# hritikbharucha/Custom_Porechop_ABI

Measured on AMD Instinct MI355X. Metric: reads/sec trimmed (100k ONT reads x 50 adapter pairs), higher is better.
Workload: dtype int32

## Files before the change

custom_porechop_abi_amd/csrc/pcabi_dp.h:

```cpp
#pragma once

#ifndef PCABI_ROW_FENCE
#define PCABI_ROW_FENCE 1
#endif
#ifndef PCABI_TAB_PD
#define PCABI_TAB_PD 0
#endif
#ifndef PCABI_TAB_PD_LONG
#define PCABI_TAB_PD_LONG 1
#endif

#include <stdint.h>
#include <algorithm>

#ifdef __HIPCC__
#define PCABI_HD __host__ __device__ __forceinline__
#else
#define PCABI_HD inline
#endif

namespace pcabi {

constexpr int NEG = -(1 << 28);

// ... 450 lines not shown
    st.best.b.trail = 0;
    st.best.b.precd = 0;
    st.best.c = -L;
    st.best.n = 0;
    st.bc = st.best;
    st.bc.b.score = SCORE_FLOOR;
    st.cslt = LT_NONE;
    st.cvt = 0;
    st.cvp = 0;
#pragma unroll 1
    for (int k = k0; k < nst; ++k) {
        adp.load(k);
        const bool first = k == k0, fin = k == nst - 1;
        const int off = first ? pad - k0 * R : 0;
        const int ib = k * R - pad;
        st.init_stripe(ib, off);
        ReadFn rd = rd0;
        BndCell up, nx, bot;
        auto row0 = [](int j, BndCell &u) { u.s = 0; u.v = NEG; u.sc = j; u.vc = 0; u.sn = 0; u.vn = 0; };
        if (first) row0(1, up);
        else bnd.load(1, up);
        int r = rd(1);
#pragma unroll 1
        for (int j = 1; j < n; ++j) {
            const int rn = rd(j + 1);
            if (first) row0(j + 1, nx);
            else bnd.load(j + 1, nx);
            st.template column<false>(r, j, up, adp, off, ib, L, fin, j >= own_lo && j < hi, sc, bot);
            if (!fin) bnd.store(j, bot);
            up = nx;
            r = rn;
        }
        if (fin_read) st.template column<true>(r, n, up, adp, off, ib, L, fin, n >= own_lo && n < hi, sc, bot);
        else st.template column<false>(r, n, up, adp, off, ib, L, fin, n >= own_lo && n < hi, sc, bot);
        if (!fin) bnd.store(n, bot);
    }
    return finish_path(st.best.b, st.best.c, (int)(st.best.n & 0xFFFFu), (int)(st.best.n >> 16), L,
                       fin_read ? n : n + 1);
}

}

namespace pcabi {

constexpr uint32_t INC_PAD = 1u << ATTR_CSH;

PCABI_HD int32_t vreg(int32_t x) {
#if defined(__HIP_DEVICE_COMPILE__)
    asm volatile("" : "+v"(x));
#endif
    return x;
}

PCABI_HD int max3i(int a, int b, int c) {
    const int ab = a > b ? a : b;
    return ab > c ? ab : c;
}
constexpr int PAD_CODE = 5;

template <int RPL, bool AFFINE>
struct LaneDP {
    int S[RPL + 1], H[RPL + 1];
    uint32_t SA[RPL + 1], HA[RPL + 1];
    int bscore, bi, bj, blt, btrail, bprec;
    uint32_t battr;
    int slt_last, ht_last, hp_last;
    int mis[4];
    uint32_t ids[4];

    template <typename AdpFn, bool LAST>
    PCABI_HD void column(const int r, const int j, const AdpFn &adp, const int L, const int off,
                         const Scoring &sc) {
        int sup = 0, vup = NEG;
        uint32_t saup = attr_start(j), vaup = 0;
        int slt_up = LT_NONE, vt_up = 0, vp_up = 0;
        int lv = 0, lh = 0, ls = 0, lslt = LT_D;
        bool lhext = false;
        uint32_t lva = 0, lha = 0, lsa = 0;
        bool match = (r == adp(1));
        int diag = 0 + (match ? sc.ma : mis[1]);
        uint32_t da = attr_start(j - 1) + ids[1] + (uint32_t)match;
#pragma unroll
        for (int s = 1; s <= RPL; ++s) {
            int diag_nx = 0;
            uint32_t da_nx = 0;
            if (s < RPL) {
                const bool mt = (r == adp(s + 1));
                const int mi_n = (s + 1 <= 3) ? mis[s + 1] : sc.mi;
                const uint32_t id_n = (s + 1 <= 3) ? ids[s + 1] : INC_D;
                diag_nx = S[s] + (mt ? sc.ma : mi_n);
                da_nx = SA[s] + id_n + (uint32_t)mt;
            }
            int hn, vn, sn;
            uint32_t han, van;
            bool hext, vext, fromv;
            if (AFFINE) {
                const int hx = H[s] + sc.ge, ho = S[s] + sc.go;
                hext = !(hx < ho);
                hn = hext ? hx : ho;
                han = hext ? HA[s] : SA[s];
                const int vx = vup + sc.ge, vo = sup + sc.go;
                vext = !(vx < vo);
                vn = vext ? vx : vo;
                van = vext ? vaup : saup;
            } else {
                hext = vext = false;
// ... 567 lines not shown
    }
    n_fin = n;
    if (CHUNK && own_hi >= 0) {
        st.template column<decltype(tabfn(r)), false, true>(tabfn(r), n, L, off, n >= own_lo && n < hi);
        st.materialize(L);
        n_fin = n + 1;
    } else {
        st.materialize(L);
        st.template column<decltype(tabfn(r)), true>(tabfn(r), n, L, off);
    }
    Best b;
    b.score = st.bscore; b.bi = st.bi; b.bj = st.bj; b.attr = Y::to_std(st.battr, st.bj);
    b.ltype = st.blt; b.trail = st.btrail; b.precd = st.bprec;
    return b;
}

template <int RPL, bool AFFINE, bool CHUNK = false, typename Y = pk::Lay<RPL>, typename ReadFn, typename TabFn>
PCABI_HD Result align_lane_packed(ReadFn &rd, int n, const TabFn &tabfn, int L, const Scoring sc, int own_lo = 1,
                                  int own_hi = -1) {
    int n_fin;
    const Best b = packed_best<RPL, AFFINE, CHUNK, Y>(rd, n, tabfn, L, sc, own_lo, own_hi, n_fin);
    return finish(b, L, n_fin);
}

namespace pk {
template <int RPL, typename AdpFn>
PCABI_HD int32_t sub_key_shift(int s, int c, const AdpFn &adp, int off, const Scoring &sc) {
    using Y = LayS<RPL>;
    if (s <= off) return Y::TD_K + Y::sc(-sc.go - sc.ge);
    return (c == adp(s)) ? (Y::sc(sc.ma - sc.go - sc.ge) + Y::TD_K + Y::INC_M)
                         : (Y::sc(sc.mi - sc.go - sc.ge) + Y::TD_K + Y::INC_D);
}
template <typename TabRow>
struct ShiftRow {
    TabRow t;
    int32_t d;
    PCABI_HD int32_t operator()(int s) const { return addw(t(s), d); }
    PCABI_HD void quad(int q, int32_t *dst) const {
        t.quad(q, dst);
        for (int k = 0; k < 4; ++k) dst[k] = addw(dst[k], d);
    }
};
}

template <int RPL, int PD = PCABI_TAB_PD>
struct LaneShift {
    using Y = pk::LayS<RPL>;
    LanePacked<RPL, true, pk::LayT<RPL>, PD> st;
    int32_t kgo;
    int32_t ftop;
    int32_t k_e;
    int32_t k_eR;
    int32_t k_rb;
    int jj, P;

    PCABI_HD void init(int L, const Scoring &sc, int P_, int B) {
        using pk::addw;
        const int off = RPL - L;
        P = P_;
        jj = 0;
        k_e = Y::sc(-sc.ge);
        k_eR = Y::sc(-sc.ge * RPL);
        k_rb = Y::sc(sc.ge * P);
        ftop = Y::sc(-B);
        kgo = Y::sc(sc.go - sc.ge) + ((P - 1) << Y::TB_SH);
        int32_t fs = addw(ftop, kgo);
#pragma unroll
        for (int s = 1; s <= RPL; ++s) {
            fs = addw(fs, k_e);
            st.G[s] = addw(Y::start(off - s), fs);
            st.HK[s] = addw(fs, Y::sc(-1) + Y::TAG1);
        }
        st.bkey = Y::start(-L);
        st.bj = 0;
    }

    PCABI_HD void advance() {
        using pk::addw;
        ++jj;
        kgo -= Y::TAG1;
        ftop = addw(ftop, k_e);
        if (jj == P) {
            const int32_t rb = addw(k_rb, P << Y::TB_SH);
#pragma unroll
            for (int s = 1; s <= RPL; ++s) {
                st.G[s] = addw(st.G[s], rb);
                st.HK[s] = addw(st.HK[s], rb);
            }
            jj = 0;
            kgo += P << Y::TB_SH;
            ftop = addw(ftop, k_rb);
        }
    }

    template <typename TabRow>
    PCABI_HD void column(const TabRow &tab, const int j, const int off) {
        using pk::addw;
        const int32_t kg = vreg(kgo);
        const int32_t top = addw(ftop, kgo);
        int32_t gup = addw(Y::start(j + off), top);
        int32_t vup = Y::SENT;
        int32_t diag = addw(addw(Y::start(j - 1 + off), top), Y::TAG1 - k_e);
        constexpr int NQ = RPL / 4;
        int32_t t[RPL + 2];
        if (PD > 0) {
#pragma unroll
            for (int q = 0; q <= PD && q < NQ; ++q) tab.quad(q, t + 4 * q + 1);
        }
        diag += (PD > 0 ? t[1] : tab(1));
        int32_t lv = 0, ls = 0;
#pragma unroll
        for (int s = 1; s <= RPL; ++s) {
            if (PD > 0 && (s & 3) == 1) {
                const int q = (s - 1) / 4 + PD + 1;
                if (q < NQ) tab.quad(q, t + 4 * q + 1);
            }
            int32_t diag_nx = 0;
            if (s < RPL) diag_nx = st.G[s] + (PD > 0 ? t[s + 1] : tab(s + 1));
            const int32_t hn = std::max(st.HK[s], st.G[s]);
            const int32_t vo = gup + Y::kv(s);
            const int32_t vn = std::max(vup, vo);
            const int32_t sn = max3i(diag, vn, hn);
            if (s == RPL) { lv = vn; ls = sn; }
            st.G[s] = (sn & ~Y::TAGM) + kg;
            st.HK[s] = hn;
            gup = st.G[s];
            vup = vn;
            diag = diag_nx;
#if defined(__HIP_DEVICE_COMPILE__)
            if (PCABI_ROW_FENCE > 0 && (s % (PCABI_ROW_FENCE > 0 ? PCABI_ROW_FENCE : 1)) == 0) __builtin_amdgcn_sched_barrier(0);
#endif
        }
        const int32_t corr = addw(std::max(lv, ls & ~Y::TAGM), pk::negw(addw(ftop, k_eR)));
        const bool upd = corr > (st.bkey | ((1 << Y::SC_SH) - 1));
        st.bkey = upd ? corr : st.bkey;
        st.bj = upd ? j : st.bj;
    }

    PCABI_HD void to_layt(const Scoring &sc) {
        using pk::addw;
        using pk::negw;
        const int32_t tagA = kgo - Y::sc(sc.go - sc.ge);
        int32_t cg = addw(negw(addw(ftop, kgo)), Y::sc(sc.go));
        int32_t ch = negw(addw(ftop, tagA + Y::TAG1));
#pragma unroll
        for (int s = 1; s <= RPL; ++s) {
            cg = addw(cg, negw(k_e));
            ch = addw(ch, negw(k_e));
            st.G[s] = addw(st.G[s], cg);
            st.HK[s] = addw(st.HK[s], ch);
        }
    }
};

template <int RPL, int PD = PCABI_TAB_PD, typename ReadFn, typename TabFn>
PCABI_HD Result align_lane_shift(ReadFn &rd, int n, const TabFn &tabfn, int L, const Scoring sc, int P, int B) {
    using Y = pk::LayS<RPL>;
    LaneShift<RPL, PD> ls;
    const int off = RPL - L;
    ls.init(L, sc, P, B);
    int r = rd(1);
#pragma unroll 1
    for (int j = 1; j < n; ++j) {
        const int rn = rd(j + 1);
        ls.advance();
        ls.template column<decltype(tabfn(r))>(tabfn(r), j, off);
        r = rn;
    }
    ls.to_layt(sc);
    auto &st = ls.st;
    const int32_t neg = Y::sc(pk::neg_score(sc));
    st.k_ge = vreg(Y::sc(sc.ge));
    st.k_go = vreg(Y::sc(sc.go));
    st.k_gev = st.k_geh = 0;
    st.k_gex = vreg(Y::sc(sc.ge) + Y::TB1);
    st.k_vo = Y::TB2;
    st.neg2 = neg | Y::TB2;
    st.materialize(L);
    const pk::ShiftRow<decltype(tabfn(r))> row{tabfn(r), Y::sc(sc.ge) + ((127 - Y::TDS) << Y::TB_SH)};
    st.template column<decltype(row), true>(row, n, L, off);
    Best b;
    b.score = st.bscore; b.bi = st.bi; b.bj = st.bj; b.attr = Y::to_std(st.battr, st.bj);
    b.ltype = st.blt; b.trail = st.btrail; b.precd = st.bprec;
    return finish(b, L, n);
}

template <int RPL, bool AFFINE, bool CHUNK = false, typename ReadFn, typename TabFn0, typename TabFn1>
PCABI_HD Result align_lane_packed_long(ReadFn &rd0, ReadFn &rd1, int n, const TabFn0 &tab0, const TabFn1 &tab1,
                                       int L, const Scoring sc, int own_lo = 1, int own_hi = -1) {
    int n_fin;
    Best b = packed_best<RPL, AFFINE, CHUNK, pk::LayL<RPL, 0>, PCABI_TAB_PD_LONG>(rd0, n, tab0, L, sc, own_lo, own_hi,
                                                                                 n_fin);
    const Best bm = packed_best<RPL, AFFINE, CHUNK, pk::LayL<RPL, 1>, PCABI_TAB_PD_LONG>(rd1, n, tab1, L, sc, own_lo,
                                                                                        own_hi, n_fin);
    b.attr |= bm.attr;
    return finish(b, L, n_fin);
}

struct SplitIn {
    int32_t gup, vup;
    int slt, vt, vp;
    int score, bi, lt, trail, prec;
    uint32_t attr;
};

template <int R, bool AFFINE, typename LAY>
struct LaneSplit {
    using Y = LAY;
    int32_t G[R + 1];
    int32_t HK[R + 1];
    int r0, off, L;
    bool last;
    int32_t k_go, k_ge, k_gex, k_vo, k_gev, k_geh, neg2;
    int32_t gdiag;
    int32_t bkey;
    int bj;
    int bscore, bi, blt, btrail, bprec;
    uint32_t battr;
    int slt_last, ht_last, hp_last;
    int32_t gbot, vbot;
    SplitIn out;
// ... 338 lines not shown
```

custom_porechop_abi_amd/csrc/pcabi_k_group.hip:

```cpp
#include "pcabi_kern.h"

namespace pcabi_eng {

template <int CLS>
__global__ __launch_bounds__(256) void k_align_group(GroupParams gp) {
    constexpr int MAXR = group_max_rpl(CLS);
    __shared__ __attribute__((aligned(16))) int32_t tab[4 * kTabW * MAXR];
    int32_t *wave_tab = tab + (threadIdx.x >> 6) * kTabW * MAXR;
    const int64_t b = blockIdx.x;
    int s = 0;
    while (s + 1 < gp.n_seg && b >= gp.seg[s + 1].block0) ++s;
    const GroupSeg &g = gp.seg[s];
    KParams p{};
    p.tiles = g.tiles;
    p.tile_off = g.tile_off;
    p.win_len = g.win_len;
    p.n_win = g.n_win;
    p.adp_pad = g.adp_pad;
    p.adp_len = g.adp_len;
    p.adp_id = g.adp_id;
    p.n_adp = g.n_adp;
    p.out = g.out;
    p.out_stride = g.out_stride;
    p.sc = gp.sc;
    p.shift_p = g.shift_p;
    p.shift_b = g.shift_b;
    const int64_t lb = b - g.block0;
    if constexpr (CLS == 0) {
        if (g.shift_p > 0) {
            switch (g.rpl) {
#define T(R) case R: cross_block<R, true, SHIFT>(p, lb, wave_tab); break;
            T(4) T(8) T(12) T(16) T(20) T(24) T(28) T(32)
#undef T
            }
        } else {
            switch (g.rpl) {
#define T(R) case R: cross_block<R, true, TAGGED>(p, lb, wave_tab); break;
            T(4) T(8) T(12) T(16) T(20) T(24) T(28) T(32)
#undef T
            }
        }
    } else {
        switch (g.rpl) {
#define P(R) case R: cross_block<R, true, PACKED>(p, lb, wave_tab); break;
        P(36) P(40) P(44) P(48) P(52) P(56) P(60) P(64)
#undef P
        }
    }
}

void dispatch_group(int cls, const GroupParams &p, int64_t blocks, hipStream_t st) {
    if (blocks <= 0) return;
    if (cls == 0) hipLaunchKernelGGL((k_align_group<0>), dim3((unsigned)blocks), dim3(256), 0, st, p);
    else hipLaunchKernelGGL((k_align_group<1>), dim3((unsigned)blocks), dim3(256), 0, st, p);
}

}
```

custom_porechop_abi_amd/csrc/pcabi_kern.h:

```cpp
#pragma once
#include <hip/hip_runtime.h>

#include <algorithm>
#include <cstdint>
#include <cstdlib>
#include <string>
#include <type_traits>

#include "../../include/pcabi.h"
#include "pcabi_dp.h"

#ifndef PCABI_WAVES
#define PCABI_WAVES 1
#endif

void pcabi_poison(void *p, size_t bytes);
void pcabi_poison_async(void *p, size_t bytes, hipStream_t st);

namespace pcabi_eng {

int fail(int code, const std::string &msg);

#define HIP_TRY(expr)                                                                   \
    do {                                                                                \
// ... 101 lines not shown

constexpr int kTabW = pcabi::pk::TAB_W;

struct LdsRow {
    const int32_t *p;
    __device__ __forceinline__ int32_t operator()(int s) const { return p[s - 1]; }
    __device__ __forceinline__ void quad(int q, int32_t *dst) const {
        const int4 v = *reinterpret_cast<const int4 *>(p + 4 * q);
        dst[0] = v.x; dst[1] = v.y; dst[2] = v.z; dst[3] = v.w;
    }
};

template <int RPL, typename Y = pcabi::pk::Lay<RPL>>
__device__ __forceinline__ void fill_wave_tab(const KParams &p, int a_local, int L, int32_t *wave_tab) {
    const int off = RPL - L;
    const int lane = threadIdx.x & 63;
    for (int e = lane; e < kTabW * RPL; e += 64) {
        const int c = e / RPL, srow = e % RPL + 1;
        const uint32_t *ap = p.adp_pad + (int64_t)a_local * (RPL / 4);
        auto code = [&](int sl) { return (int)((ap[(sl - 1) / 4] >> (8 * ((sl - 1) & 3))) & 0xFFu); };
        wave_tab[e] = pcabi::pk::sub_key<RPL, decltype(code), Y>(srow, c, code, off, p.sc);
    }
    __syncthreads();
}

template <int RPL>
__device__ __forceinline__ void fill_wave_tab_shift(const KParams &p, int a_local, int L, int32_t *wave_tab) {
    const int off = RPL - L;
    const int lane = threadIdx.x & 63;
    for (int e = lane; e < kTabW * RPL; e += 64) {
        const int c = e / RPL, srow = e % RPL + 1;
        const uint32_t *ap = p.adp_pad + (int64_t)a_local * (RPL / 4);
        auto code = [&](int sl) { return (int)((ap[(sl - 1) / 4] >> (8 * ((sl - 1) & 3))) & 0xFFu); };
        wave_tab[e] = pcabi::pk::sub_key_shift<RPL>(srow, c, code, off, p.sc);
    }
    __syncthreads();
}

template <int RPL>
__device__ __forceinline__ void fill_wave_tab_long(const KParams &p, int a_local, int L, int32_t *wave_tab) {
    const int off = RPL - L;
    const int lane = threadIdx.x & 63;
    const uint32_t *ap = p.adp_pad + (int64_t)a_local * (RPL / 4);
    auto code = [&](int sl) { return (int)((ap[(sl - 1) / 4] >> (8 * ((sl - 1) & 3))) & 0xFFu); };
    for (int e = lane; e < kTabW * RPL; e += 64) {
        const int c = e / RPL, srow = e % RPL + 1;
        wave_tab[e] = pcabi::pk::sub_key<RPL, decltype(code), pcabi::pk::LayL<RPL, 0>>(srow, c, code, off, p.sc);
        wave_tab[kTabW * RPL + e] =
            pcabi::pk::sub_key<RPL, decltype(code), pcabi::pk::LayL<RPL, 1>>(srow, c, code, off, p.sc);
    }
    __syncthreads();
}

template <int RPL, bool AFFINE, int KIND>
__device__ __forceinline__ void run_lane(const KParams &p, int a_local, int64_t w, int64_t out_idx,
                                         int32_t *wave_tab, int64_t tile_off) {
    AdapterRegs<RPL> adp;
    if constexpr (KIND != LONG) adp.load(p.adp_pad + (int64_t)a_local * (RPL / 4));
    const int L = __builtin_amdgcn_readfirstlane(p.adp_len[a_local]);
    if constexpr (KIND == PACKED) fill_wave_tab<RPL>(p, a_local, L, wave_tab);
    if constexpr (KIND == TAGGED) fill_wave_tab<RPL, pcabi::pk::LayT<RPL>>(p, a_local, L, wave_tab);
    if constexpr (KIND == SHIFT) fill_wave_tab_shift<RPL>(p, a_local, L, wave_tab);
    if constexpr (KIND == LONG) fill_wave_tab_long<RPL>(p, a_local, L, wave_tab);
    if (w < 0) return;
    const int n = p.win_len[w];
    pcabi::Result r;
    if (n <= 0) {
        r = empty_result();
    } else {
        WindowReader rd = tile_off >= 0
            ? WindowReader(p.tiles + tile_off + (threadIdx.x & 255), 256, 0)
            : [&] {
                  const uint8_t *b = p.codes + p.win_off[w];
                  const int a0 = (int)((uintptr_t)b & 3);
                  return WindowReader(reinterpret_cast<const uint32_t *>(b - a0), 1, 8 * a0);
              }();
        if constexpr (KIND == PACKED) {
            auto tabfn = [&](int rc) { return LdsRow{wave_tab + rc * RPL}; };
            r = pcabi::align_lane_packed<(RPL <= pcabi::pk::MAX_RPL ? RPL : 4), AFFINE>(rd, n, tabfn, L, p.sc);
        } else if constexpr (KIND == TAGGED) {
            static_assert(RPL <= 32 && AFFINE, "run-tagged layout: affine buckets of <= 32 rows");
            auto tabfn = [&](int rc) { return LdsRow{wave_tab + rc * RPL}; };
            r = pcabi::align_lane_packed<RPL, true, false, pcabi::pk::LayT<RPL>>(rd, n, tabfn, L, p.sc);
        } else if constexpr (KIND == SHIFT) {
            static_assert(RPL <= 32 && AFFINE, "gap-extend frame: affine buckets of <= 32 rows");
            auto tabfn = [&](int rc) { return LdsRow{wave_tab + rc * RPL}; };
            r = pcabi::align_lane_shift<RPL>(rd, n, tabfn, L, p.sc, p.shift_p, p.shift_b);
        } else if constexpr (KIND == LONG) {
            WindowReader rd1 = rd;
            auto tab0 = [&](int rc) { return LdsRow{wave_tab + rc * RPL}; };
            auto tab1 = [&](int rc) { return LdsRow{wave_tab + kTabW * RPL + rc * RPL}; };
            r = pcabi::align_lane_packed_long<RPL, AFFINE>(rd, rd1, n, tab0, tab1, L, p.sc);
        } else if constexpr (KIND == FAST) {
            r = pcabi::align_lane_fast<RPL, AFFINE>(rd, n, adp, L, p.sc);
        } else {
            r = pcabi::align_lane_generic<RPL, AFFINE>(rd, n, adp, L, p.sc);
        }
    }
    if (p.compat) {
        int en_match = 0;
        if (r.rs >= 0 && r.diag_en && r.l1 > 0) {
            const uint8_t *ab = reinterpret_cast<const uint8_t *>(p.adp_pad + (int64_t)a_local * (RPL / 4));
            en_match = p.codes[p.win_off[w] + r.re] == ab[RPL - L + r.ae];
        }
        p.compat[out_idx] = pcabi::compat_flag(r, n, en_match);
        return;
    }
    store_result(p.out, p.out_stride, out_idx, r);
}

template <int KIND, int RPL>
constexpr int wave_tab_ints() {
    return (KIND == PACKED || KIND == TAGGED || KIND == SHIFT) ? kTabW * RPL : (KIND == LONG ? 2 * kTabW * RPL : 1);
}

template <int RPL, bool AFFINE, int KIND>
__device__ __forceinline__ void cross_block(const KParams &p, int64_t b, int32_t *wave_tab) {
    const int64_t k = b >> 3;
    const int a_local = (int)(k % p.n_adp);
    const int64_t tile = (k / p.n_adp) * 8 + (b & 7);
    const int64_t w = tile * 256 + threadIdx.x;
    const int a_glob = p.adp_id[a_local];
    const int64_t toff = w < p.n_win ? p.tile_off[tile] : 0;
    run_lane<RPL, AFFINE, KIND>(p, a_local, w < p.n_win ? w : -1, (int64_t)a_glob * p.n_win + w, wave_tab, toff);
}

template <int RPL, bool AFFINE, int KIND>
__global__ __launch_bounds__(256, PCABI_WAVES) void k_align(KParams p) {
    __shared__ __attribute__((aligned(16))) int32_t tab[4 * wave_tab_ints<KIND, RPL>()];
    int32_t *wave_tab = tab + (threadIdx.x >> 6) * wave_tab_ints<KIND, RPL>();
    if (p.task_win == nullptr) {
        cross_block<RPL, AFFINE, KIND>(p, blockIdx.x, wave_tab);
    } else {
        int64_t wave = (int64_t)blockIdx.x * 4 + (threadIdx.x >> 6);
        const bool live = wave < p.n_waves;
        if (!live) wave = p.n_waves - 1;
        const int64_t slot = wave * 64 + (threadIdx.x & 63);
        const int a_local = __builtin_amdgcn_readfirstlane(p.wave_adp[wave]);
        const int32_t tw = live ? p.task_win[slot] : -1;
        run_lane<RPL, AFFINE, KIND>(p, a_local, tw, tw >= 0 ? p.task_out[slot] : 0, wave_tab, -1);
    }
}

struct FParams {
    const uint32_t *tiles;
    const int64_t *tile_off;
    const int32_t *win_len;
    int64_t n_win;
    const uint32_t *adp_pad;
    const int32_t *adp_len;
    const int32_t *adp_id;
    int32_t n_adp;
    int16_t *s16;
    pcabi::Scoring sc;
};

struct LdsRow16 {
    const int32_t *p;
    __device__ __forceinline__ void quad(int q, pcabi::sf::v2 *dst) const {
        const int4 v = *reinterpret_cast<const int4 *>(p + 4 * q);
        dst[0] = __builtin_bit_cast(pcabi::sf::v2, v.x);
        dst[1] = __builtin_bit_cast(pcabi::sf::v2, v.y);
        dst[2] = __builtin_bit_cast(pcabi::sf::v2, v.z);
        dst[3] = __builtin_bit_cast(pcabi::sf::v2, v.w);
    }
};

template <int RPL, bool AFFINE>
__global__ __launch_bounds__(256) void k_score_filter(FParams p) {
    __shared__ __attribute__((aligned(16))) int32_t tab[4 * kTabW * RPL];
    int32_t *wave_tab = tab + (threadIdx.x >> 6) * kTabW * RPL;
    const int n_pair = (p.n_adp + 1) / 2;
    const int64_t b = blockIdx.x;
    const int64_t k = b >> 3;
    const int pr = (int)(k % n_pair);
    const int64_t tile = (k / n_pair) * 8 + (b & 7);
    const int64_t w = tile * 256 + threadIdx.x;
// ... 400 lines not shown
```

Baseline: 16.36 million.

## Defer best-cell tracking to per-period merge and add wave-uniform loop path

The per-column best-score update in the shift-frame DP becomes a single max3 into a running packed key, with the column offset encoded in tag bits. It is merged into the global best only once per rebase period and after the loop. The SHIFT kernel also checks with a ballot whether all lanes share the same read length. When they do, it runs a scalar-trip-count loop instead of an exec-mask loop, which removes per-iteration vector compares and exec manipulation. The cost is more intricate tag arithmetic, a risk of edge-case errors in index recovery, and two code paths.

```diff
diff --git a/custom_porechop_abi_amd/csrc/pcabi_dp.h b/custom_porechop_abi_amd/csrc/pcabi_dp.h
--- a/custom_porechop_abi_amd/csrc/pcabi_dp.h
+++ b/custom_porechop_abi_amd/csrc/pcabi_dp.h
@@ -526,6 +526,13 @@
     return x;
 }
 
+PCABI_HD int wave_uniform(int x) {
+#if defined(__HIP_DEVICE_COMPILE__)
+    x = __builtin_amdgcn_readfirstlane(x);
+#endif
+    return x;
+}
+
 PCABI_HD int max3i(int a, int b, int c) {
     const int ab = a > b ? a : b;
     return ab > c ? ab : c;
@@ -1199,18 +1206,24 @@
     int32_t k_e;
     int32_t k_eR;
     int32_t k_rb;
+    int32_t ksc;
+    int32_t pbest;
+    int jbase;
     int jj, P;
 
     PCABI_HD void init(int L, const Scoring &sc, int P_, int B) {
         using pk::addw;
         const int off = RPL - L;
         P = P_;
-        jj = 0;
+        jj = -1;
+        jbase = 1;
+        pbest = Y::SENT;
         k_e = Y::sc(-sc.ge);
         k_eR = Y::sc(-sc.ge * RPL);
         k_rb = Y::sc(sc.ge * P);
-        ftop = Y::sc(-B);
-        kgo = Y::sc(sc.go - sc.ge) + ((P - 1) << Y::TB_SH);
+        ftop = addw(Y::sc(-B), pk::negw(k_e));
+        kgo = Y::sc(sc.go - sc.ge) + (P << Y::TB_SH);
+        ksc = addw(pk::negw(addw(ftop, k_eR)), (2 * P) << Y::TB_SH);
         int32_t fs = addw(ftop, kgo);
 #pragma unroll
         for (int s = 1; s <= RPL; ++s) {
@@ -1227,7 +1240,9 @@
         ++jj;
         kgo -= Y::TAG1;
         ftop = addw(ftop, k_e);
+        ksc = addw(ksc, pk::negw(k_e) - 2 * Y::TAG1);
         if (jj == P) {
+            merge();
             const int32_t rb = addw(k_rb, P << Y::TB_SH);
 #pragma unroll
             for (int s = 1; s <= RPL; ++s) {
@@ -1235,9 +1250,19 @@
                 st.HK[s] = addw(st.HK[s], rb);
             }
             jj = 0;
+            jbase += P;
             kgo += P << Y::TB_SH;
             ftop = addw(ftop, k_rb);
-        }
+            ksc = addw(ksc, addw(pk::negw(k_rb), (2 * P) << Y::TB_SH));
+        }
+    }
+
+    PCABI_HD void merge() {
+        const bool upd = pbest > (st.bkey | ((1 << Y::SC_SH) - 1));
+        const int a = (pbest >> (Y::TB_SH + 1)) & 63;
+        st.bkey = upd ? (pbest & ~(Y::TAGM - Y::TAG1)) : st.bkey;
+        st.bj = upd ? jbase + P - 1 - a : st.bj;
+        pbest = Y::SENT;
     }
 
     template <typename TabRow>
@@ -1278,10 +1303,7 @@
             if (PCABI_ROW_FENCE > 0 && (s % (PCABI_ROW_FENCE > 0 ? PCABI_ROW_FENCE : 1)) == 0) __builtin_amdgcn_sched_barrier(0);
 #endif
         }
-        const int32_t corr = addw(std::max(lv, ls & ~Y::TAGM), pk::negw(addw(ftop, k_eR)));
-        const bool upd = corr > (st.bkey | ((1 << Y::SC_SH) - 1));
-        st.bkey = upd ? corr : st.bkey;
-        st.bj = upd ? j : st.bj;
+        pbest = max3i(pbest, addw(lv & ~Y::TAGM, ksc + Y::TAG1), addw(ls & ~Y::TAGM, ksc));
     }
 
     PCABI_HD void to_layt(const Scoring &sc) {
@@ -1301,19 +1323,28 @@
 };
 
 template <int RPL, int PD = PCABI_TAB_PD, typename ReadFn, typename TabFn>
-PCABI_HD Result align_lane_shift(ReadFn &rd, int n, const TabFn &tabfn, int L, const Scoring sc, int P, int B) {
+PCABI_HD Result align_lane_shift(ReadFn &rd, int n, const TabFn &tabfn, int L, const Scoring sc, int P, int B,
+                                 bool uni = false) {
     using Y = pk::LayS<RPL>;
     LaneShift<RPL, PD> ls;
     const int off = RPL - L;
     ls.init(L, sc, P, B);
     int r = rd(1);
-#pragma unroll 1
-    for (int j = 1; j < n; ++j) {
+    auto step = [&](int j) {
         const int rn = rd(j + 1);
         ls.advance();
         ls.template column<decltype(tabfn(r))>(tabfn(r), j, off);
         r = rn;
-    }
+    };
+    if (uni) {
+        const int nu = wave_uniform(n);
+#pragma unroll 1
+        for (int j = 1; j < nu; ++j) step(j);
+    } else {
+#pragma unroll 1
+        for (int j = 1; j < n; ++j) step(j);
+    }
+    ls.merge();
     ls.to_layt(sc);
     auto &st = ls.st;
     const int32_t neg = Y::sc(pk::neg_score(sc));
diff --git a/custom_porechop_abi_amd/csrc/pcabi_k_group.hip b/custom_porechop_abi_amd/csrc/pcabi_k_group.hip
--- a/custom_porechop_abi_amd/csrc/pcabi_k_group.hip
+++ b/custom_porechop_abi_amd/csrc/pcabi_k_group.hip
@@ -1,6 +1,8 @@
 #include "pcabi_kern.h"
 
 namespace pcabi_eng {
+
+constexpr int kUniLoopMaxRows = 28;
 
 template <int CLS>
 __global__ __launch_bounds__(256) void k_align_group(GroupParams gp) {
@@ -29,7 +31,7 @@
     if constexpr (CLS == 0) {
         if (g.shift_p > 0) {
             switch (g.rpl) {
-#define T(R) case R: cross_block<R, true, SHIFT>(p, lb, wave_tab); break;
+#define T(R) case R: cross_block<R, true, SHIFT, (R <= kUniLoopMaxRows)>(p, lb, wave_tab); break;
             T(4) T(8) T(12) T(16) T(20) T(24) T(28) T(32)
 #undef T
             }
diff --git a/custom_porechop_abi_amd/csrc/pcabi_kern.h b/custom_porechop_abi_amd/csrc/pcabi_kern.h
--- a/custom_porechop_abi_amd/csrc/pcabi_kern.h
+++ b/custom_porechop_abi_amd/csrc/pcabi_kern.h
@@ -177,7 +177,7 @@
     __syncthreads();
 }
 
-template <int RPL, bool AFFINE, int KIND>
+template <int RPL, bool AFFINE, int KIND, bool UNILOOP = false>
 __device__ __forceinline__ void run_lane(const KParams &p, int a_local, int64_t w, int64_t out_idx,
                                          int32_t *wave_tab, int64_t tile_off) {
     AdapterRegs<RPL> adp;
@@ -210,7 +210,8 @@
         } else if constexpr (KIND == SHIFT) {
             static_assert(RPL <= 32 && AFFINE, "gap-extend frame: affine buckets of <= 32 rows");
             auto tabfn = [&](int rc) { return LdsRow{wave_tab + rc * RPL}; };
-            r = pcabi::align_lane_shift<RPL>(rd, n, tabfn, L, p.sc, p.shift_p, p.shift_b);
+            const bool uni = UNILOOP && __builtin_amdgcn_ballot_w64(n != __builtin_amdgcn_readfirstlane(n)) == 0;
+            r = pcabi::align_lane_shift<RPL>(rd, n, tabfn, L, p.sc, p.shift_p, p.shift_b, uni);
         } else if constexpr (KIND == LONG) {
             WindowReader rd1 = rd;
             auto tab0 = [&](int rc) { return LdsRow{wave_tab + rc * RPL}; };
@@ -239,7 +240,7 @@
     return (KIND == PACKED || KIND == TAGGED || KIND == SHIFT) ? kTabW * RPL : (KIND == LONG ? 2 * kTabW * RPL : 1);
 }
 
-template <int RPL, bool AFFINE, int KIND>
+template <int RPL, bool AFFINE, int KIND, bool UNILOOP = false>
 __device__ __forceinline__ void cross_block(const KParams &p, int64_t b, int32_t *wave_tab) {
     const int64_t k = b >> 3;
     const int a_local = (int)(k % p.n_adp);
@@ -247,7 +248,8 @@
     const int64_t w = tile * 256 + threadIdx.x;
     const int a_glob = p.adp_id[a_local];
     const int64_t toff = w < p.n_win ? p.tile_off[tile] : 0;
-    run_lane<RPL, AFFINE, KIND>(p, a_local, w < p.n_win ? w : -1, (int64_t)a_glob * p.n_win + w, wave_tab, toff);
+    run_lane<RPL, AFFINE, KIND, UNILOOP>(p, a_local, w < p.n_win ? w : -1, (int64_t)a_glob * p.n_win + w, wave_tab,
+                                         toff);
 }
 
 template <int RPL, bool AFFINE, int KIND>
diff --git a/profiles/r08/k_align_group0_24row_lane_column.s b/profiles/r08/k_align_group0_24row_lane_column.s
--- /dev/null
+++ b/profiles/r08/k_align_group0_24row_lane_column.s
@@ -0,0 +1,329 @@
+.LBB0_757:
+	s_and_b32 s4, s53, 24
+	v_lshrrev_b64 v[64:65], s4, v[10:11]
+	s_movk_i32 s4, 0x60
+	v_mov_b32_e32 v70, v31
+	v_mad_u32_u24 v31, v68, s4, v12
+	v_mov_b32_e32 v68, s47
+	ds_read_b64 v[66:67], v31
+	s_and_b32 vcc_lo, s51, 0x1fc00
+	s_add_i32 s4, s46, s47
+	s_add_i32 s62, s51, 0xfffe0400
+	s_sub_i32 vcc_lo, vcc_lo, s42
+	s_and_b32 s62, s62, 0x1fc00
+	s_add_i32 vcc_lo, s4, vcc_lo
+	s_add_i32 vcc_lo, vcc_lo, 0x20000
+	s_add_i32 s4, s4, s62
+	s_waitcnt lgkmcnt(0)
+	v_add_u32_e32 v66, vcc_lo, v66
+	v_max_i32_e32 v60, v60, v4
+	s_add_i32 s4, s4, 0xbe0000
+	v_add_u32_e32 v67, v67, v4
+	v_max3_i32 v4, v66, s4, v60
+	v_and_b32_e32 v4, 0xff01ffff, v4
+	v_and_b32_e32 v64, 0xff, v64
+	v_mov_b32_e32 v65, s47
+	v_add_u32_e32 v4, v4, v68
+	ds_read_b32 v66, v31 offset:8
+	v_add_u32_e32 v72, 0xbc0000, v4
+	v_max_i32_e32 v59, v59, v57
+	v_max_i32_e32 v72, s4, v72
+	v_max3_i32 v67, v67, v72, v59
+	s_waitcnt lgkmcnt(0)
+	v_add_u32_e32 v66, v66, v57
+	v_and_b32_e32 v57, 0xff01ffff, v67
+	v_add_u32_e32 v57, v57, v68
+	ds_read_b32 v67, v31 offset:12
+	v_add_u32_e32 v73, 0xba0000, v57
+	v_max_i32_e32 v58, v58, v55
+	v_max_i32_e32 v72, v72, v73
+	v_max3_i32 v66, v66, v72, v58
+	s_waitcnt lgkmcnt(0)
+	v_add_u32_e32 v67, v67, v55
+	v_and_b32_e32 v55, 0xff01ffff, v66
+	v_add_u32_e32 v55, v55, v68
+	ds_read_b32 v66, v31 offset:16
+	v_add_u32_e32 v73, 0xb80000, v55
+	v_max_i32_e32 v56, v56, v53
+	v_max_i32_e32 v72, v72, v73
+	v_max3_i32 v67, v67, v72, v56
+	s_waitcnt lgkmcnt(0)
+	v_add_u32_e32 v66, v66, v53
+	v_and_b32_e32 v53, 0xff01ffff, v67
+	v_add_u32_e32 v53, v53, v68
+	ds_read_b32 v67, v31 offset:20
+	v_add_u32_e32 v73, 0xb60000, v53
+	v_max_i32_e32 v54, v54, v51
+	v_max_i32_e32 v72, v72, v73
+	v_max3_i32 v66, v66, v72, v54
+	s_waitcnt lgkmcnt(0)
+	v_add_u32_e32 v67, v67, v51
+	v_and_b32_e32 v51, 0xff01ffff, v66
+	v_add_u32_e32 v51, v51, v68
+	ds_read_b32 v66, v31 offset:24
+	v_add_u32_e32 v73, 0xb40000, v51
+	v_max_i32_e32 v52, v52, v49
+	v_max_i32_e32 v72, v72, v73
+	v_max3_i32 v67, v67, v72, v52
+	s_waitcnt lgkmcnt(0)
+	v_add_u32_e32 v66, v66, v49
+	v_and_b32_e32 v49, 0xff01ffff, v67
+	v_add_u32_e32 v49, v49, v68
+	ds_read_b32 v67, v31 offset:28
+	v_add_u32_e32 v73, 0xb20000, v49
+	v_max_i32_e32 v50, v50, v47
+	v_max_i32_e32 v72, v72, v73
+	v_max3_i32 v66, v66, v72, v50
+	s_waitcnt lgkmcnt(0)
+	v_add_u32_e32 v67, v67, v47
+	v_and_b32_e32 v47, 0xff01ffff, v66
+	v_add_u32_e32 v47, v47, v68
+	ds_read_b32 v66, v31 offset:32
+	v_add_u32_e32 v73, 0xb00000, v47
+	v_max_i32_e32 v48, v48, v45
+	v_max_i32_e32 v72, v72, v73
+	v_max3_i32 v67, v67, v72, v48
+	s_waitcnt lgkmcnt(0)
+	v_add_u32_e32 v66, v66, v45
+	v_and_b32_e32 v45, 0xff01ffff, v67
+	v_add_u32_e32 v45, v45, v68
+	ds_read_b32 v67, v31 offset:36
+	v_add_u32_e32 v73, 0xae0000, v45
+	v_max_i32_e32 v46, v46, v43
+	v_max_i32_e32 v72, v72, v73
+	v_max3_i32 v66, v66, v72, v46
+	s_waitcnt lgkmcnt(0)
+	v_add_u32_e32 v67, v67, v43
+	v_and_b32_e32 v43, 0xff01ffff, v66
+	v_add_u32_e32 v43, v43, v68
+	ds_read_b32 v66, v31 offset:40
+	v_add_u32_e32 v73, 0xac0000, v43
+	v_max_i32_e32 v44, v44, v41
+	v_max_i32_e32 v72, v72, v73
+	v_max3_i32 v67, v67, v72, v44
+	s_waitcnt lgkmcnt(0)
+	v_add_u32_e32 v66, v66, v41
+	v_and_b32_e32 v41, 0xff01ffff, v67
+	v_add_u32_e32 v41, v41, v68
+	ds_read_b32 v67, v31 offset:44
+	v_add_u32_e32 v73, 0xaa0000, v41
+	v_max_i32_e32 v42, v42, v39
+	v_max_i32_e32 v72, v72, v73
+	v_max3_i32 v66, v66, v72, v42
+	s_waitcnt lgkmcnt(0)
+	v_add_u32_e32 v67, v67, v39
+	v_and_b32_e32 v39, 0xff01ffff, v66
+	v_add_u32_e32 v39, v39, v68
+	ds_read_b32 v66, v31 offset:48
+	v_add_u32_e32 v73, 0xa80000, v39
+	v_max_i32_e32 v40, v40, v37
+	v_max_i32_e32 v72, v72, v73
+	v_max3_i32 v67, v67, v72, v40
+	s_waitcnt lgkmcnt(0)
+	v_add_u32_e32 v66, v66, v37
+	v_and_b32_e32 v37, 0xff01ffff, v67
+	v_add_u32_e32 v37, v37, v68
+	ds_read_b32 v67, v31 offset:52
+	v_add_u32_e32 v73, 0xa60000, v37
+	v_max_i32_e32 v38, v38, v35
+	v_max_i32_e32 v72, v72, v73
+	v_max3_i32 v66, v66, v72, v38
+	s_waitcnt lgkmcnt(0)
+	v_add_u32_e32 v67, v67, v35
+	v_and_b32_e32 v35, 0xff01ffff, v66
+	v_add_u32_e32 v35, v35, v68
+	ds_read_b32 v66, v31 offset:56
+	v_add_u32_e32 v73, 0xa40000, v35
+	v_max_i32_e32 v36, v36, v33
+	v_max_i32_e32 v72, v72, v73
+	v_max3_i32 v67, v67, v72, v36
+	s_waitcnt lgkmcnt(0)
+	v_add_u32_e32 v66, v66, v33
+	v_and_b32_e32 v33, 0xff01ffff, v67
+	v_add_u32_e32 v33, v33, v68
+	ds_read_b32 v67, v31 offset:60
+	v_add_u32_e32 v73, 0xa20000, v33
+	v_max_i32_e32 v34, v34, v30
+	v_max_i32_e32 v72, v72, v73
+	v_max3_i32 v66, v66, v72, v34
+	s_waitcnt lgkmcnt(0)
+	v_add_u32_e32 v67, v67, v30
+	v_and_b32_e32 v30, 0xff01ffff, v66
+	v_add_u32_e32 v30, v30, v68
+	ds_read_b32 v66, v31 offset:64
+	v_add_u32_e32 v73, 0xa00000, v30
+	v_max_i32_e32 v32, v32, v28
+	v_max_i32_e32 v72, v72, v73
+	v_max3_i32 v67, v67, v72, v32
+	s_waitcnt lgkmcnt(0)
+	v_add_u32_e32 v66, v66, v28
+	v_and_b32_e32 v28, 0xff01ffff, v67
+	v_add_u32_e32 v28, v28, v68
+	ds_read_b32 v67, v31 offset:68
+	v_add_u32_e32 v73, 0x9e0000, v28
+	v_max_i32_e32 v29, v29, v26
+	v_max_i32_e32 v72, v72, v73
+	v_max3_i32 v66, v66, v72, v29
+	s_waitcnt lgkmcnt(0)
+	v_add_u32_e32 v67, v67, v26
+	v_and_b32_e32 v26, 0xff01ffff, v66
+	v_add_u32_e32 v26, v26, v68
+	ds_read_b32 v66, v31 offset:72
+	v_add_u32_e32 v73, 0x9c0000, v26
+	v_max_i32_e32 v27, v27, v24
+	v_max_i32_e32 v72, v72, v73
+	v_max3_i32 v67, v67, v72, v27
+	s_waitcnt lgkmcnt(0)
+	v_add_u32_e32 v66, v66, v24
+	v_and_b32_e32 v24, 0xff01ffff, v67
+	v_add_u32_e32 v24, v24, v68
+	ds_read_b32 v67, v31 offset:76
+	v_add_u32_e32 v73, 0x9a0000, v24
+	v_max_i32_e32 v25, v25, v22
+	v_max_i32_e32 v72, v72, v73
+	v_max3_i32 v66, v66, v72, v25
+	s_waitcnt lgkmcnt(0)
+	v_add_u32_e32 v67, v67, v22
+	v_and_b32_e32 v22, 0xff01ffff, v66
+	v_add_u32_e32 v22, v22, v68
+	ds_read_b32 v66, v31 offset:80
+	v_add_u32_e32 v73, 0x980000, v22
+	v_max_i32_e32 v23, v23, v20
+	v_max_i32_e32 v72, v72, v73
+	v_max3_i32 v67, v67, v72, v23
+	s_waitcnt lgkmcnt(0)
+	v_add_u32_e32 v66, v66, v20
+	v_and_b32_e32 v20, 0xff01ffff, v67
+	v_add_u32_e32 v20, v20, v68
+	ds_read_b32 v67, v31 offset:84
+	v_add_u32_e32 v73, 0x960000, v20
+	v_max_i32_e32 v21, v21, v18
+	v_max_i32_e32 v72, v72, v73
+	v_max3_i32 v66, v66, v72, v21
+	s_waitcnt lgkmcnt(0)
+	v_add_u32_e32 v67, v67, v18
+	v_and_b32_e32 v18, 0xff01ffff, v66
+	v_add_u32_e32 v18, v18, v68
+	ds_read_b32 v66, v31 offset:88
+	v_add_u32_e32 v73, 0x940000, v18
+	v_max_i32_e32 v19, v19, v16
+	v_max_i32_e32 v72, v72, v73
+	v_max3_i32 v67, v67, v72, v19
+	s_waitcnt lgkmcnt(0)
+	v_add_u32_e32 v66, v66, v16
+	v_and_b32_e32 v16, 0xff01ffff, v67
+	v_add_u32_e32 v16, v16, v68
+	ds_read_b32 v67, v31 offset:92
+	v_add_u32_e32 v31, 0x920000, v16
+	v_max_i32_e32 v17, v17, v70
+	v_max_i32_e32 v72, v72, v31
+	v_max3_i32 v31, v66, v72, v17
+	v_and_b32_e32 v31, 0xff01ffff, v31
+	v_add_u32_e32 v31, v31, v68
+	v_max_i32_e32 v15, v15, v14
+	v_add_u32_e32 v14, 0x900000, v31
+	s_waitcnt lgkmcnt(0)
+	v_add_u32_e32 v66, v67, v70
+	v_max_i32_e32 v67, v72, v14
+	v_max3_i32 v14, v66, v67, v15
+	v_and_b32_e32 v66, 0xff01ffff, v14
+	v_add_u32_e32 v14, v66, v68
+	v_and_b32_e32 v67, 0xff01ffff, v67
+	s_add_i32 s4, s50, 0x20000
+	s_add_i32 s52, s52, 1
+	v_add_u32_e32 v67, s4, v67
+	v_add_u32_e32 v66, s50, v66
+	s_addk_i32 s51, 0x400
+	s_add_i32 s53, s53, 8
+	v_cmp_eq_u32_e32 vcc, s52, v13
+	v_max3_i32 v61, v61, v67, v66
+	s_or_b64 s[2:3], vcc, s[2:3]
+	v_mov_b32_e32 v67, s46
+	v_mov_b32_e32 v66, s54
+	s_mov_b32 s4, s5
+	v_mov_b32_e32 v68, v64
+	s_andn2_b64 exec, exec, s[2:3]
+	s_cbranch_execz .LBB0_778
+.LBB0_758:
+	s_and_b32 s5, s52, 3
+	s_cmp_lg_u32 s5, 0
+	s_cbranch_scc1 .LBB0_760
+	s_lshr_b32 s5, s52, 2
+	s_add_i32 s62, s5, 2
+	s_lshl_b64 vcc, s[62:63], 10
+	v_mov_b32_e32 v70, v11
+	v_lshl_add_u64 v[64:65], v[6:7], 0, vcc
+	s_waitcnt vmcnt(0)
+	v_mov_b64_e32 v[10:11], v[70:71]
+	global_load_dword v71, v[64:65], off
+.LBB0_760:
+	s_sub_i32 s50, s50, s42
+	s_add_i32 s5, s4, 1
+	s_add_i32 s47, s47, 0xfffe0000
+	s_add_i32 s46, s46, s42
+	s_add_i32 s50, s50, 0xfffc0000
+	s_cmp_lg_u32 s5, s30
+	s_cbranch_scc1 .LBB0_757
+	v_or_b32_e32 v64, 0xffffff, v62
+	v_and_b32_e32 v65, 0xff03ffff, v61
+	v_cmp_gt_i32_e32 vcc, v61, v64
+	v_bfe_u32 v61, v61, 18, 6
+	s_add_i32 s4, s54, s4
+	v_sub_u32_e32 v61, s4, v61
+	v_cndmask_b32_e32 v62, v62, v65, vcc
+	v_cndmask_b32_e32 v5, v5, v61, vcc
+	v_add_u32_e32 v4, s49, v4
+	v_add_u32_e32 v60, s49, v60
+	v_add_u32_e32 v57, s49, v57
+	v_add_u32_e32 v59, s49, v59
+	v_add_u32_e32 v55, s49, v55
+	v_add_u32_e32 v58, s49, v58
+	v_add_u32_e32 v53, s49, v53
+	v_add_u32_e32 v56, s49, v56
+	v_add_u32_e32 v51, s49, v51
+	v_add_u32_e32 v54, s49, v54
+	v_add_u32_e32 v49, s49, v49
+	v_add_u32_e32 v52, s49, v52
+	v_add_u32_e32 v47, s49, v47
+	v_add_u32_e32 v50, s49, v50
+	v_add_u32_e32 v45, s49, v45
+	v_add_u32_e32 v48, s49, v48
+	v_add_u32_e32 v43, s49, v43
+	v_add_u32_e32 v46, s49, v46
+	v_add_u32_e32 v41, s49, v41
+	v_add_u32_e32 v44, s49, v44
+	v_add_u32_e32 v39, s49, v39
+	v_add_u32_e32 v42, s49, v42
+	v_add_u32_e32 v37, s49, v37
+	v_add_u32_e32 v40, s49, v40
+	v_add_u32_e32 v35, s49, v35
+	v_add_u32_e32 v38, s49, v38
+	v_add_u32_e32 v33, s49, v33
+	v_add_u32_e32 v36, s49, v36
+	v_add_u32_e32 v30, s49, v30
+	v_add_u32_e32 v34, s49, v34
+	v_add_u32_e32 v28, s49, v28
+	v_add_u32_e32 v32, s49, v32
+	v_add_u32_e32 v26, s49, v26
+	v_add_u32_e32 v29, s49, v29
+	v_add_u32_e32 v24, s49, v24
+	v_add_u32_e32 v27, s49, v27
+	v_add_u32_e32 v22, s49, v22
+	v_add_u32_e32 v25, s49, v25
+	v_add_u32_e32 v20, s49, v20
+	v_add_u32_e32 v23, s49, v23
+	v_add_u32_e32 v18, s49, v18
+	v_add_u32_e32 v21, s49, v21
+	v_add_u32_e32 v16, s49, v16
+	v_add_u32_e32 v19, s49, v19
+	v_add_u32_e32 v31, s49, v31
+	v_add_u32_e32 v17, s49, v17
+	v_add_u32_e32 v14, s49, v14
+	v_add_u32_e32 v15, s49, v15
+	s_add_i32 s54, s54, s30
+	s_add_i32 s47, s47, s34
+	s_add_i32 s46, s46, s48
+	s_add_i32 s50, s35, s50
+	s_mov_b32 s5, 0
+	v_bfrev_b32_e32 v61, 1
+	s_branch .LBB0_757
diff --git a/profiles/r08/k_align_group0_24row_uniform_column.s b/profiles/r08/k_align_group0_24row_uniform_column.s
--- /dev/null
+++ b/profiles/r08/k_align_group0_24row_uniform_column.s
@@ -0,0 +1,326 @@
+.LBB0_783:
+	v_or_b32_e32 v10, 0xffffff, v62
+	v_cmp_gt_i32_e32 vcc, v61, v10
+	v_bfe_u32 v10, v61, 18, 6
+	s_add_i32 s0, s2, s46
+	v_and_b32_e32 v11, 0xff03ffff, v61
+	v_sub_u32_e32 v10, s0, v10
+	v_cndmask_b32_e32 v62, v62, v11, vcc
+	v_cndmask_b32_e32 v5, v5, v10, vcc
+	v_add_u32_e32 v4, s4, v4
+	v_add_u32_e32 v60, s4, v60
+	v_add_u32_e32 v57, s4, v57
+	v_add_u32_e32 v59, s4, v59
+	v_add_u32_e32 v55, s4, v55
+	v_add_u32_e32 v58, s4, v58
+	v_add_u32_e32 v53, s4, v53
+	v_add_u32_e32 v56, s4, v56
+	v_add_u32_e32 v51, s4, v51
+	v_add_u32_e32 v54, s4, v54
+	v_add_u32_e32 v49, s4, v49
+	v_add_u32_e32 v52, s4, v52
+	v_add_u32_e32 v47, s4, v47
+	v_add_u32_e32 v50, s4, v50
+	v_add_u32_e32 v45, s4, v45
+	v_add_u32_e32 v48, s4, v48
+	v_add_u32_e32 v43, s4, v43
+	v_add_u32_e32 v46, s4, v46
+	v_add_u32_e32 v41, s4, v41
+	v_add_u32_e32 v44, s4, v44
+	v_add_u32_e32 v39, s4, v39
+	v_add_u32_e32 v42, s4, v42
+	v_add_u32_e32 v37, s4, v37
+	v_add_u32_e32 v40, s4, v40
+	v_add_u32_e32 v35, s4, v35
+	v_add_u32_e32 v38, s4, v38
+	v_add_u32_e32 v33, s4, v33
+	v_add_u32_e32 v36, s4, v36
+	v_add_u32_e32 v30, s4, v30
+	v_add_u32_e32 v34, s4, v34
+	v_add_u32_e32 v28, s4, v28
+	v_add_u32_e32 v32, s4, v32
+	v_add_u32_e32 v26, s4, v26
+	v_add_u32_e32 v29, s4, v29
+	v_add_u32_e32 v24, s4, v24
+	v_add_u32_e32 v27, s4, v27
+	v_add_u32_e32 v22, s4, v22
+	v_add_u32_e32 v25, s4, v25
+	v_add_u32_e32 v20, s4, v20
+	v_add_u32_e32 v23, s4, v23
+	v_add_u32_e32 v18, s4, v18
+	v_add_u32_e32 v21, s4, v21
+	v_add_u32_e32 v16, s4, v16
+	v_add_u32_e32 v19, s4, v19
+	v_add_u32_e32 v31, s4, v31
+	v_add_u32_e32 v17, s4, v17
+	v_add_u32_e32 v14, s4, v14
+	v_add_u32_e32 v15, s4, v15
+	s_add_i32 s2, s2, s30
+	s_add_i32 s58, s58, s34
+	s_add_i32 s56, s56, s48
+	s_add_i32 s55, s5, s55
+	s_mov_b32 s46, 0
+	v_bfrev_b32_e32 v61, 1
+.LBB0_784:
+	s_and_b32 s0, s51, 24
+	s_waitcnt vmcnt(1)
+	v_lshrrev_b64 v[10:11], s0, v[8:9]
+	v_mad_u32_u24 v11, v63, s40, v12
+	v_mov_b32_e32 v63, s58
+	ds_read_b64 v[64:65], v11
+	s_and_b32 s45, s35, 0x1fc00
+	s_add_i32 s0, s56, s58
+	s_add_i32 s41, s35, 0xfffe0400
+	s_sub_i32 s45, s45, s42
+	s_and_b32 s41, s41, 0x1fc00
+	s_add_i32 s45, s0, s45
+	s_add_i32 s45, s45, 0x20000
+	s_add_i32 s0, s0, s41
+	v_mov_b32_e32 v66, v31
+	s_waitcnt lgkmcnt(0)
+	v_add_u32_e32 v31, s45, v64
+	v_max_i32_e32 v60, v60, v4
+	s_add_i32 s0, s0, 0xbe0000
+	v_add_u32_e32 v64, v65, v4
+	v_max3_i32 v4, v31, s0, v60
+	v_and_b32_e32 v4, 0xff01ffff, v4
+	v_add_u32_e32 v4, v4, v63
+	v_and_b32_e32 v10, 0xff, v10
+	ds_read_b32 v31, v11 offset:8
+	v_add_u32_e32 v65, 0xbc0000, v4
+	v_max_i32_e32 v59, v59, v57
+	v_max_i32_e32 v65, s0, v65
+	v_max3_i32 v64, v64, v65, v59
+	s_waitcnt lgkmcnt(0)
+	v_add_u32_e32 v31, v31, v57
+	v_and_b32_e32 v57, 0xff01ffff, v64
+	v_add_u32_e32 v57, v57, v63
+	ds_read_b32 v64, v11 offset:12
+	v_add_u32_e32 v67, 0xba0000, v57
+	v_max_i32_e32 v58, v58, v55
+	v_max_i32_e32 v65, v65, v67
+	v_max3_i32 v31, v31, v65, v58
+	v_and_b32_e32 v31, 0xff01ffff, v31
+	s_waitcnt lgkmcnt(0)
+	v_add_u32_e32 v64, v64, v55
+	v_add_u32_e32 v55, v31, v63
+	ds_read_b32 v31, v11 offset:16
+	v_add_u32_e32 v67, 0xb80000, v55
+	v_max_i32_e32 v56, v56, v53
+	v_max_i32_e32 v65, v65, v67
+	v_max3_i32 v64, v64, v65, v56
+	s_waitcnt lgkmcnt(0)
+	v_add_u32_e32 v31, v31, v53
+	v_and_b32_e32 v53, 0xff01ffff, v64
+	v_add_u32_e32 v53, v53, v63
+	ds_read_b32 v64, v11 offset:20
+	v_add_u32_e32 v67, 0xb60000, v53
+	v_max_i32_e32 v54, v54, v51
+	v_max_i32_e32 v65, v65, v67
+	v_max3_i32 v31, v31, v65, v54
+	v_and_b32_e32 v31, 0xff01ffff, v31
+	s_waitcnt lgkmcnt(0)
+	v_add_u32_e32 v64, v64, v51
+	v_add_u32_e32 v51, v31, v63
+	ds_read_b32 v31, v11 offset:24
+	v_add_u32_e32 v67, 0xb40000, v51
+	v_max_i32_e32 v52, v52, v49
+	v_max_i32_e32 v65, v65, v67
+	v_max3_i32 v64, v64, v65, v52
+	s_waitcnt lgkmcnt(0)
+	v_add_u32_e32 v31, v31, v49
+	v_and_b32_e32 v49, 0xff01ffff, v64
+	v_add_u32_e32 v49, v49, v63
+	ds_read_b32 v64, v11 offset:28
+	v_add_u32_e32 v67, 0xb20000, v49
+	v_max_i32_e32 v50, v50, v47
+	v_max_i32_e32 v65, v65, v67
+	v_max3_i32 v31, v31, v65, v50
+	v_and_b32_e32 v31, 0xff01ffff, v31
+	s_waitcnt lgkmcnt(0)
+	v_add_u32_e32 v64, v64, v47
+	v_add_u32_e32 v47, v31, v63
+	ds_read_b32 v31, v11 offset:32
+	v_add_u32_e32 v67, 0xb00000, v47
+	v_max_i32_e32 v48, v48, v45
+	v_max_i32_e32 v65, v65, v67
+	v_max3_i32 v64, v64, v65, v48
+	s_waitcnt lgkmcnt(0)
+	v_add_u32_e32 v31, v31, v45
+	v_and_b32_e32 v45, 0xff01ffff, v64
+	v_add_u32_e32 v45, v45, v63
+	ds_read_b32 v64, v11 offset:36
+	v_add_u32_e32 v67, 0xae0000, v45
+	v_max_i32_e32 v46, v46, v43
+	v_max_i32_e32 v65, v65, v67
+	v_max3_i32 v31, v31, v65, v46
+	v_and_b32_e32 v31, 0xff01ffff, v31
+	s_waitcnt lgkmcnt(0)
+	v_add_u32_e32 v64, v64, v43
+	v_add_u32_e32 v43, v31, v63
+	ds_read_b32 v31, v11 offset:40
+	v_add_u32_e32 v67, 0xac0000, v43
+	v_max_i32_e32 v44, v44, v41
+	v_max_i32_e32 v65, v65, v67
+	v_max3_i32 v64, v64, v65, v44
+	s_waitcnt lgkmcnt(0)
+	v_add_u32_e32 v31, v31, v41
+	v_and_b32_e32 v41, 0xff01ffff, v64
+	v_add_u32_e32 v41, v41, v63
+	ds_read_b32 v64, v11 offset:44
+	v_add_u32_e32 v67, 0xaa0000, v41
+	v_max_i32_e32 v42, v42, v39
+	v_max_i32_e32 v65, v65, v67
+	v_max3_i32 v31, v31, v65, v42
+	v_and_b32_e32 v31, 0xff01ffff, v31
+	s_waitcnt lgkmcnt(0)
+	v_add_u32_e32 v64, v64, v39
+	v_add_u32_e32 v39, v31, v63
+	ds_read_b32 v31, v11 offset:48
+	v_add_u32_e32 v67, 0xa80000, v39
+	v_max_i32_e32 v40, v40, v37
+	v_max_i32_e32 v65, v65, v67
+	v_max3_i32 v64, v64, v65, v40
+	s_waitcnt lgkmcnt(0)
+	v_add_u32_e32 v31, v31, v37
+	v_and_b32_e32 v37, 0xff01ffff, v64
+	v_add_u32_e32 v37, v37, v63
+	ds_read_b32 v64, v11 offset:52
+	v_add_u32_e32 v67, 0xa60000, v37
+	v_max_i32_e32 v38, v38, v35
+	v_max_i32_e32 v65, v65, v67
+	v_max3_i32 v31, v31, v65, v38
+	v_and_b32_e32 v31, 0xff01ffff, v31
+	s_waitcnt lgkmcnt(0)
+	v_add_u32_e32 v64, v64, v35
+	v_add_u32_e32 v35, v31, v63
+	ds_read_b32 v31, v11 offset:56
+	v_add_u32_e32 v67, 0xa40000, v35
+	v_max_i32_e32 v36, v36, v33
+	v_max_i32_e32 v65, v65, v67
+	v_max3_i32 v64, v64, v65, v36
+	s_waitcnt lgkmcnt(0)
+	v_add_u32_e32 v31, v31, v33
+	v_and_b32_e32 v33, 0xff01ffff, v64
+	v_add_u32_e32 v33, v33, v63
+	ds_read_b32 v64, v11 offset:60
+	v_add_u32_e32 v67, 0xa20000, v33
+	v_max_i32_e32 v34, v34, v30
+	v_max_i32_e32 v65, v65, v67
+	v_max3_i32 v31, v31, v65, v34
+	s_waitcnt lgkmcnt(0)
+	v_add_u32_e32 v64, v64, v30
+	v_and_b32_e32 v30, 0xff01ffff, v31
+	v_add_u32_e32 v30, v30, v63
+	ds_read_b32 v31, v11 offset:64
+	v_add_u32_e32 v67, 0xa00000, v30
+	v_max_i32_e32 v32, v32, v28
+	v_max_i32_e32 v65, v65, v67
+	v_max3_i32 v64, v64, v65, v32
+	s_waitcnt lgkmcnt(0)
+	v_add_u32_e32 v31, v31, v28
+	v_and_b32_e32 v28, 0xff01ffff, v64
+	v_add_u32_e32 v28, v28, v63
+	ds_read_b32 v64, v11 offset:68
+	v_add_u32_e32 v67, 0x9e0000, v28
+	v_max_i32_e32 v29, v29, v26
+	v_max_i32_e32 v65, v65, v67
+	v_max3_i32 v31, v31, v65, v29
+	s_waitcnt lgkmcnt(0)
+	v_add_u32_e32 v64, v64, v26
+	v_and_b32_e32 v26, 0xff01ffff, v31
+	v_add_u32_e32 v26, v26, v63
+	ds_read_b32 v31, v11 offset:72
+	v_add_u32_e32 v67, 0x9c0000, v26
+	v_max_i32_e32 v27, v27, v24
+	v_max_i32_e32 v65, v65, v67
+	v_max3_i32 v64, v64, v65, v27
+	s_waitcnt lgkmcnt(0)
+	v_add_u32_e32 v31, v31, v24
+	v_and_b32_e32 v24, 0xff01ffff, v64
+	v_add_u32_e32 v24, v24, v63
+	ds_read_b32 v64, v11 offset:76
+	v_add_u32_e32 v67, 0x9a0000, v24
+	v_max_i32_e32 v25, v25, v22
+	v_max_i32_e32 v65, v65, v67
+	v_max3_i32 v31, v31, v65, v25
+	s_waitcnt lgkmcnt(0)
+	v_add_u32_e32 v64, v64, v22
+	v_and_b32_e32 v22, 0xff01ffff, v31
+	v_add_u32_e32 v22, v22, v63
+	ds_read_b32 v31, v11 offset:80
+	v_add_u32_e32 v67, 0x980000, v22
+	v_max_i32_e32 v23, v23, v20
+	v_max_i32_e32 v65, v65, v67
+	v_max3_i32 v64, v64, v65, v23
+	s_waitcnt lgkmcnt(0)
+	v_add_u32_e32 v31, v31, v20
+	v_and_b32_e32 v20, 0xff01ffff, v64
+	v_add_u32_e32 v20, v20, v63
+	ds_read_b32 v64, v11 offset:84
+	v_add_u32_e32 v67, 0x960000, v20
+	v_max_i32_e32 v21, v21, v18
+	v_max_i32_e32 v65, v65, v67
+	v_max3_i32 v31, v31, v65, v21
+	s_waitcnt lgkmcnt(0)
+	v_add_u32_e32 v64, v64, v18
+	v_and_b32_e32 v18, 0xff01ffff, v31
+	v_add_u32_e32 v18, v18, v63
+	ds_read_b32 v31, v11 offset:88
+	v_add_u32_e32 v67, 0x940000, v18
+	v_max_i32_e32 v19, v19, v16
+	v_max_i32_e32 v65, v65, v67
+	v_max3_i32 v64, v64, v65, v19
+	s_waitcnt lgkmcnt(0)
+	v_add_u32_e32 v31, v31, v16
+	v_and_b32_e32 v16, 0xff01ffff, v64
+	v_add_u32_e32 v16, v16, v63
+	v_add_u32_e32 v64, 0x920000, v16
+	ds_read_b32 v11, v11 offset:92
+	v_max_i32_e32 v17, v17, v66
+	v_max_i32_e32 v64, v65, v64
+	v_max3_i32 v31, v31, v64, v17
+	v_and_b32_e32 v31, 0xff01ffff, v31
+	v_add_u32_e32 v31, v31, v63
+	v_max_i32_e32 v15, v15, v14
+	v_add_u32_e32 v14, 0x900000, v31
+	s_waitcnt lgkmcnt(0)
+	v_add_u32_e32 v11, v11, v66
+	v_max_i32_e32 v64, v64, v14
+	v_max3_i32 v11, v11, v64, v15
+	v_and_b32_e32 v11, 0xff01ffff, v11
+	v_add_u32_e32 v14, v11, v63
+	v_and_b32_e32 v63, 0xff01ffff, v64
+	s_add_i32 s0, s55, 0x20000
+	v_add_u32_e32 v63, s0, v63
+	v_add_u32_e32 v11, s55, v11
+	s_add_i32 s49, s49, 1
+	s_addk_i32 s35, 0x400
+	s_add_i32 s51, s51, 8
+	s_cmp_eq_u32 s3, s49
+	v_max3_i32 v61, v61, v63, v11
+	v_mov_b32_e32 v63, v10
+	s_cbranch_scc1 .LBB0_801
+.LBB0_785:
+	s_and_b32 s0, s49, 3
+	s_cmp_lg_u32 s0, 0
+	s_cbranch_scc1 .LBB0_787
+	s_lshr_b32 s0, s49, 2
+	s_add_i32 s0, s0, 2
+	s_lshl_b64 s[52:53], s[0:1], 10
+	s_waitcnt vmcnt(1)
+	v_mov_b32_e32 v68, v9
+	v_lshl_add_u64 v[10:11], v[6:7], 0, s[52:53]
+	s_waitcnt vmcnt(0)
+	v_mov_b64_e32 v[8:9], v[68:69]
+	global_load_dword v69, v[10:11], off
+.LBB0_787:
+	s_sub_i32 s41, s55, s42
+	s_add_i32 s0, s46, 1
+	s_add_i32 s58, s58, 0xfffe0000
+	s_add_i32 s56, s56, s42
+	s_add_i32 s55, s41, 0xfffc0000
+	s_cmp_lg_u32 s0, s30
+	s_cbranch_scc0 .LBB0_783
+	s_mov_b32 s46, s0
+	s_branch .LBB0_784
```

After: 16.70 million (median of 6 runs). 1.02x the previous value.
